# ZiyuanMa/MAPF_RL

Measured on NVIDIA B200. Metric: env_agent_steps_per_sec_step_observe, higher is better.
Workload: dtype u8

## Files before the change

mapf_rl_b200/csrc/mapf_bfs_device.cuh:

```cuda
#pragma once
#include <type_traits>

#include "mapf_common.cuh"

namespace {

#ifdef MAPF_ENABLE_DIAG
__device__ unsigned long long g_bfs_cycles[8];
#endif

template <int RW, int RPL>
struct BfsState {
    uint32_t unv[RPL][RW];
    uint32_t fro[RPL][RW];
    uint32_t m1[RPL][RW];
    uint32_t m2[RPL][RW];
};

__device__ __forceinline__ uint32_t bfs_column_mask(int L, int w)
{
    const int lo = max(4 - 32 * w, 0), hi = min(L + 4 - 32 * w, 32);
    if (hi <= lo) return 0u;
    return (hi - lo == 32) ? 0xffffffffu : (((1u << (hi - lo)) - 1u) << lo);
}

template <int RW, int RPL>
struct BfsFree {
    uint32_t v[RPL][RW];
};

template <int RW, int RPL, int APW>
__device__ __forceinline__ void bfs_load_free(const EnvDims &d, const uint32_t *ob, BfsFree<RW, RPL> &F)
{
    constexpr int LW = 32 / APW;
    const int lane = (threadIdx.x & 31) % LW;
#pragma unroll
    for (int q = 0; q < RPL; ++q) {
        const int row = lane * RPL + q;
#pragma unroll
        for (int w = 0; w < RW; ++w)
            F.v[q][w] = (row < d.L) ? (~__ldcg(ob + (row + 4) * d.RWS + w) & bfs_column_mask(d.L, w)) : 0u;
    }
}

template <int RW, int RPL, int APW>
__device__ __forceinline__ void bfs_init(const EnvDims &d, const BfsFree<RW, RPL> &F, const int gx, const int gy, const bool alive,
                                         BfsState<RW, RPL> &S)
{
    constexpr int LW = 32 / APW;
    const int lane = (threadIdx.x & 31) % LW;
#pragma unroll
    for (int q = 0; q < RPL; ++q) {
        const int row = lane * RPL + q;
#pragma unroll
        for (int w = 0; w < RW; ++w) {
            const uint32_t fre = alive ? F.v[q][w] : 0u;
            const int p = gy + 4;
            S.fro[q][w] = (row == gx && (p >> 5) == w) ? ((1u << (p & 31)) & fre) : 0u;
            S.unv[q][w] = fre & ~S.fro[q][w];
            S.m1[q][w] = S.m2[q][w] = 0;
        }
    }
}

template <int RW, int RPL, int APW, bool WRAP>
__device__ __forceinline__ uint32_t bfs_wave(const BfsState<RW, RPL> &S, uint32_t (&nw)[RPL][RW])
{
    constexpr int LW = 32 / APW;
    const int lane = (threadIdx.x & 31) % LW;
    uint32_t any = 0;
#pragma unroll
    for (int w = 0; w < RW; ++w) {
        uint32_t above, below;
        if constexpr (WRAP) {
            above = __shfl_sync(MAPF_FULL_MASK, S.fro[RPL - 1][w], (lane + LW - 1) & (LW - 1), LW);
            below = __shfl_sync(MAPF_FULL_MASK, S.fro[0][w], (lane + 1) & (LW - 1), LW);
        } else {
            above = __shfl_up_sync(MAPF_FULL_MASK, S.fro[RPL - 1][w], 1, LW);
            below = __shfl_down_sync(MAPF_FULL_MASK, S.fro[0][w], 1, LW);
            if (lane == 0) above = 0;
            if (lane == LW - 1) below = 0;
        }
#pragma unroll
        for (int q = 0; q < RPL; ++q) {
            const uint32_t f = S.fro[q][w];
            const uint32_t fl = w > 0 ? __funnelshift_l(S.fro[q][w > 0 ? w - 1 : 0], f, 1) : f << 1;
            const uint32_t fr = w < RW - 1 ? __funnelshift_r(f, S.fro[q][w < RW - 1 ? w + 1 : w], 1) : f >> 1;
            const uint32_t up = q > 0 ? S.fro[q > 0 ? q - 1 : 0][w] : above;
            const uint32_t dn = q < RPL - 1 ? S.fro[q < RPL - 1 ? q + 1 : q][w] : below;
            const uint32_t x = (fl | fr | up | dn) & S.unv[q][w];
            nw[q][w] = x;
            any |= x;
        }
    }
    return any;
}

template <int RW, int RPL, int SEL>
__device__ __forceinline__ void bfs_apply(BfsState<RW, RPL> &S, const uint32_t (&nw)[RPL][RW])
{
#pragma unroll
    for (int q = 0; q < RPL; ++q)
#pragma unroll
        for (int w = 0; w < RW; ++w) {
            S.unv[q][w] -= nw[q][w];
            S.fro[q][w] = nw[q][w];
            if constexpr (SEL == 1) S.m1[q][w] += nw[q][w];
            if constexpr (SEL == 2) S.m2[q][w] += nw[q][w];
        }
}

template <int RW, int RPL, int APW, bool KEEP>
__device__ __forceinline__ void bfs_emit(const EnvDims &d, const uint32_t *ob, const BfsFree<RW, RPL> &F, const int e, const int a,
                                         const bool alive, const BfsState<RW, RPL> &S, uint32_t *__restrict__ navi)
{
    constexpr int LW = 32 / APW;
    const int lane = (threadIdx.x & 31) % LW;
    uint32_t pl[4][RPL][RW];
    uint32_t z[RPL][RW];
#pragma unroll
    for (int q = 0; q < RPL; ++q) {
        const int row = alive ? lane * RPL + q : d.L;
#pragma unroll
        for (int w = 0; w < RW; ++w) {
            uint32_t fre;
            if constexpr (KEEP) fre = alive ? F.v[q][w] : 0u;
            else fre = (row < d.L) ? (~__ldcg(ob + (row + 4) * d.RWS + w) & bfs_column_mask(d.L, w)) : 0u;
            z[q][w] = fre & ~S.unv[q][w] & ~S.m1[q][w] & ~S.m2[q][w];
        }
    }
    auto closer = [](uint32_t c1, uint32_t c2, uint32_t cz, uint32_t n1, uint32_t n2, uint32_t nz) -> uint32_t {
        return (c1 & nz) | (c2 & n1) | (cz & n2);
    };
#pragma unroll
    for (int w = 0; w < RW; ++w) {
        uint32_t a1 = __shfl_up_sync(MAPF_FULL_MASK, S.m1[RPL - 1][w], 1, LW), b1 = __shfl_down_sync(MAPF_FULL_MASK, S.m1[0][w], 1, LW);
        uint32_t a2 = __shfl_up_sync(MAPF_FULL_MASK, S.m2[RPL - 1][w], 1, LW), b2 = __shfl_down_sync(MAPF_FULL_MASK, S.m2[0][w], 1, LW);
        uint32_t az = __shfl_up_sync(MAPF_FULL_MASK, z[RPL - 1][w], 1, LW), bz = __shfl_down_sync(MAPF_FULL_MASK, z[0][w], 1, LW);
        if (lane == 0) a1 = a2 = az = 0;
        if (lane == LW - 1) b1 = b2 = bz = 0;
#pragma unroll
        for (int q = 0; q < RPL; ++q) {
            auto left = [&](const uint32_t(&m)[RPL][RW]) {
                return w > 0 ? __funnelshift_l(m[q][w > 0 ? w - 1 : 0], m[q][w], 1) : m[q][w] << 1;
            };
            auto right = [&](const uint32_t(&m)[RPL][RW]) {
                return w < RW - 1 ? __funnelshift_r(m[q][w], m[q][w < RW - 1 ? w + 1 : w], 1) : m[q][w] >> 1;
            };
            const uint32_t c1 = S.m1[q][w], c2 = S.m2[q][w], cz = z[q][w];
            const uint32_t u1 = q > 0 ? S.m1[q > 0 ? q - 1 : 0][w] : a1, u2 = q > 0 ? S.m2[q > 0 ? q - 1 : 0][w] : a2,
                           uz = q > 0 ? z[q > 0 ? q - 1 : 0][w] : az;
            const uint32_t d1 = q < RPL - 1 ? S.m1[q < RPL - 1 ? q + 1 : q][w] : b1, d2 = q < RPL - 1 ? S.m2[q < RPL - 1 ? q + 1 : q][w] : b2,
                           dz = q < RPL - 1 ? z[q < RPL - 1 ? q + 1 : q][w] : bz;
            pl[0][q][w] = closer(c1, c2, cz, u1, u2, uz);
            pl[1][q][w] = closer(c1, c2, cz, d1, d2, dz);
            pl[2][q][w] = closer(c1, c2, cz, left(S.m1), left(S.m2), left(z));
            pl[3][q][w] = closer(c1, c2, cz, right(S.m1), right(S.m2), right(z));
        }
    }
    uint2 *nv = reinterpret_cast<uint2 *>(navi + ((size_t)e * d.N + a) * d.navi_agent_stride);
#pragma unroll
    for (int q = 0; q < RPL; ++q) {
        const int row = lane * RPL + q;
        if (row >= d.L || !alive) continue;
        const int pr = row + 4, bx1 = pr >> 3, r1 = pr & 7;
#pragma unroll
        for (int by = 0; by < 4 * RW; ++by) {
            if (by >= d.NB) continue;
            constexpr int kLast = RW - 1;
            const int w = by >> 2;
            const int s = (by & 3) * 8;
            uint32_t f[4];
#pragma unroll
            for (int k = 0; k < 4; ++k)
                f[k] = __funnelshift_r(pl[k][q][w], w < kLast ? pl[k][q][w < kLast ? w + 1 : kLast] : 0u, s) & 0xffffu;
            const uint2 v = make_uint2(f[0] | (f[1] << 16), f[2] | (f[3] << 16));
            if (bx1 < d.NB) nv[((size_t)(bx1 * d.NB + by) << 4) + r1] = v;
            if (bx1 > 0) nv[((size_t)((bx1 - 1) * d.NB + by) << 4) + r1 + 8] = v;
        }
    }
}

template <int RW, int RPL, int APW, bool WRAP, bool DIST, bool KEEP>
__device__ __forceinline__ void bfs_navi_search(const EnvDims &d, const int e, const int a, const int i, const bool alive,
                                                const uint32_t *__restrict__ ob, const BfsFree<RW, RPL> &F, const int gx, const int gy,
                                                uint32_t *__restrict__ navi, int32_t *__restrict__ dist_out)
{
    constexpr int LW = 32 / APW;
    const int lane = (threadIdx.x & 31) % LW;
#ifdef MAPF_ENABLE_DIAG
    const long long tb0 = clock64();
    long long triples = 0;
#endif
    BfsState<RW, RPL> S;
    bfs_init<RW, RPL, APW>(d, F, gx, gy, alive, S);
#ifdef MAPF_ENABLE_DIAG
    const long long tb1 = clock64();
#endif

    int32_t *dist = nullptr;
    if constexpr (DIST) {
        dist = alive ? dist_out + ((size_t)i * d.N + a) * d.L * d.L : nullptr;
        for (int q = 0; q < RPL; ++q) {
            const int row = lane * RPL + q;
            if (dist && row < d.L)
                for (int y = 0; y < d.L; ++y) dist[row * d.L + y] = MAPF_DIST_UNREACHABLE;
        }
        __syncwarp();
#pragma unroll
        for (int q = 0; q < RPL; ++q)
#pragma unroll
            for (int w = 0; w < RW; ++w)
                if (dist && S.fro[q][w]) dist[gx * d.L + gy] = 0;
    }

    auto wave = [&](auto selc, const int t) -> uint32_t {
        constexpr int sel = decltype(selc)::value;
        uint32_t nw[RPL][RW];
        const uint32_t any = bfs_wave<RW, RPL, APW, WRAP>(S, nw);
        bfs_apply<RW, RPL, sel>(S, nw);
        if constexpr (DIST) {
#pragma unroll
            for (int q = 0; q < RPL; ++q)
#pragma unroll
                for (int w = 0; w < RW; ++w) {
                    uint32_t x = dist ? nw[q][w] : 0u;
                    while (x) {
                        int b = __ffs(x) - 1;
                        x &= x - 1;
                        dist[(lane * RPL + q) * d.L + (32 * w + b - 4)] = t;
                    }
                }
        }
        return any;
    };
    for (int t = 1;; t += 3) {
        wave(std::integral_constant<int, 1>{}, t);
        wave(std::integral_constant<int, 2>{}, t + 1);
        const uint32_t any = wave(std::integral_constant<int, 0>{}, t + 2);
#ifdef MAPF_ENABLE_DIAG
        ++triples;
#endif
        if (!__any_sync(MAPF_FULL_MASK, any != 0)) break;
    }
#ifdef MAPF_ENABLE_DIAG
    const long long tb2 = clock64();
#endif
    bfs_emit<RW, RPL, APW, KEEP>(d, ob, F, e, a, alive, S, navi);
#ifdef MAPF_ENABLE_DIAG
    if (e == 0 && (threadIdx.x & 31) == 0) {
        const long long tb3 = clock64();
        atomicAdd(&g_bfs_cycles[0], (unsigned long long)(tb1 - tb0));
        atomicAdd(&g_bfs_cycles[1], (unsigned long long)(tb2 - tb1));
        atomicAdd(&g_bfs_cycles[2], (unsigned long long)(tb3 - tb2));
        atomicAdd(&g_bfs_cycles[3], 1ull);
        atomicAdd(&g_bfs_cycles[4], (unsigned long long)triples);
    }
#endif
}

template <int RW, int RPL, int APW>
__device__ __forceinline__ void bfs_navi_warp(const EnvDims &d, const int e, const int a, const int i, const bool alive,
                                              const uint32_t *__restrict__ obst, const uint8_t *__restrict__ goal,
                                              uint32_t *__restrict__ navi, int32_t *__restrict__ dist_out)
{
    constexpr int LW = 32 / APW;
    const uint32_t *ob = obst + (size_t)e * d.obst_stride;
    const uchar2 gg = __ldcg(reinterpret_cast<const uchar2 *>(goal) + (size_t)e * d.N + a);
    BfsFree<RW, RPL> F;
    bfs_load_free<RW, RPL, APW>(d, ob, F);
    if (dist_out) bfs_navi_search<RW, RPL, APW, false, true, false>(d, e, a, i, alive, ob, F, gg.x, gg.y, navi, dist_out);
    else if (d.L < LW * RPL) bfs_navi_search<RW, RPL, APW, true, false, false>(d, e, a, i, alive, ob, F, gg.x, gg.y, navi, nullptr);
    else bfs_navi_search<RW, RPL, APW, false, false, false>(d, e, a, i, alive, ob, F, gg.x, gg.y, navi, nullptr);
}

template <int RW, int RPL, int APW>
__device__ __forceinline__ void bfs_navi_warp_pre(const EnvDims &d, const int e, const int a, const bool alive, const uint32_t *__restrict__ ob,
                                                  const BfsFree<RW, RPL> &F, const int gx, const int gy, uint32_t *__restrict__ navi)
{
    constexpr int LW = 32 / APW;
    if (d.L < LW * RPL) bfs_navi_search<RW, RPL, APW, true, false, true>(d, e, a, 0, alive, ob, F, gx, gy, navi, nullptr);
    else bfs_navi_search<RW, RPL, APW, false, false, true>(d, e, a, 0, alive, ob, F, gx, gy, navi, nullptr);
}

}
```

mapf_rl_b200/csrc/mapf_reset_device.cuh:

```cuda
#pragma once
#include "mapf_common.cuh"

namespace {


__device__ __forceinline__ uint4 philox4x32_10(uint4 c, uint2 k)
{
#pragma unroll
    for (int r = 0; r < 10; ++r) {
        const uint32_t hi0 = __umulhi(0xD2511F53u, c.x), lo0 = 0xD2511F53u * c.x;
        const uint32_t hi1 = __umulhi(0xCD9E8D57u, c.z), lo1 = 0xCD9E8D57u * c.z;
        c = make_uint4(hi1 ^ c.y ^ k.x, lo1, hi0 ^ c.w ^ k.y, lo0);
        k.x += 0x9E3779B9u;
        k.y += 0xBB67AE85u;
    }
    return c;
}

enum : uint32_t { PURPOSE_DENSITY = 0, PURPOSE_MAP = 1, PURPOSE_AGENT = 2 };

#ifdef MAPF_ENABLE_DIAG
__device__ unsigned long long g_reset_cycles[8];
#define MAPF_RESET_TICK(slot)                 \
    do {                                      \
        const long long _now = clock64();     \
        _acc[slot] += _now - _t0;             \
        _t0 = _now;                           \
    } while (0)
#else
#define MAPF_RESET_TICK(slot) do {} while (0)
#endif

template <int RW, int RPL>
struct Bits {
    uint32_t v[RPL][RW];
};

template <int RW, int RPL>
__device__ __forceinline__ void dilate(const Bits<RW, RPL> &f, Bits<RW, RPL> &out, int lane)
{
#pragma unroll
    for (int q = 0; q < RPL; ++q)
#pragma unroll
        for (int w = 0; w < RW; ++w) {
            const uint32_t x = f.v[q][w];
            uint32_t fl = x << 1, fr = x >> 1;
            if (w > 0) fl |= f.v[q][w > 0 ? w - 1 : 0] >> 31;
            if (w < RW - 1) fr |= f.v[q][w < RW - 1 ? w + 1 : w] << 31;
            uint32_t up = __shfl_up_sync(MAPF_FULL_MASK, x, 1);
            uint32_t dn = __shfl_down_sync(MAPF_FULL_MASK, x, 1);
            uint32_t wrap_up = 0, wrap_dn = 0;
            if (q > 0) wrap_up = __shfl_sync(MAPF_FULL_MASK, f.v[q > 0 ? q - 1 : 0][w], 31);
            if (q < RPL - 1) wrap_dn = __shfl_sync(MAPF_FULL_MASK, f.v[q < RPL - 1 ? q + 1 : q][w], 0);
            if (lane == 0) up = wrap_up;
            if (lane == 31) dn = wrap_dn;
            out.v[q][w] = fl | fr | up | dn;
        }
}

template <int RW, int RPL>
__device__ __forceinline__ int count_bits(const Bits<RW, RPL> &m)
{
    int c = 0;
#pragma unroll
    for (int q = 0; q < RPL; ++q)
#pragma unroll
        for (int w = 0; w < RW; ++w) c += __popc(m.v[q][w]);
    return c;
}

__device__ __forceinline__ int nth_set_bit(uint32_t m, int n)
{
    int pos = 0;
#pragma unroll
    for (int half = 16; half >= 1; half >>= 1) {
        const int c = __popc(m & ((1u << half) - 1u));
        if (n >= c) {
            n -= c;
            pos += half;
            m >>= half;
        }
    }
    return pos;
}

template <int RW, int RPL>
__device__ __forceinline__ int pick_bit(const Bits<RW, RPL> &m, uint32_t rnd, int lane, int &total_out)
{
    constexpr int kMax = 32 * RW * RPL;
    constexpr int kBits = kMax >= 512 ? 10 : (kMax >= 256 ? 9 : (kMax >= 128 ? 8 : (kMax >= 64 ? 7 : 6)));
    const int c = count_bits(m);
    const uint32_t lt = (1u << lane) - 1u;
    int excl = 0, total = 0;
#pragma unroll
    for (int k = 0; k < kBits; ++k) {
        const uint32_t b = __ballot_sync(MAPF_FULL_MASK, (c >> k) & 1);
        excl += __popc(b & lt) << k;
        total += __popc(b) << k;
    }
    total_out = total;
    if (total == 0) return -1;
    const int r = (int)__umulhi(rnd, (uint32_t)total);
    int local = r - excl;
    uint32_t code = 0;
    if (local >= 0 && local < c) {
        bool found = false;
#pragma unroll
        for (int q = 0; q < RPL; ++q)
#pragma unroll
            for (int w = 0; w < RW; ++w) {
                const int pc = __popc(m.v[q][w]);
                if (!found && local < pc) {
                    code = (uint32_t)((((lane + 32 * q) << 8) | (32 * w + nth_set_bit(m.v[q][w], local))) + 1);
                    found = true;
                }
                if (!found) local -= pc;
            }
    }
    return (int)__reduce_or_sync(MAPF_FULL_MASK, code) - 1;
}

template <int RW, int RPL>
__device__ __forceinline__ void clear_cell(Bits<RW, RPL> &m, int code, int lane)
{
    const int row = code >> 8, col = code & 0xff;
#pragma unroll
    for (int q = 0; q < RPL; ++q)
#pragma unroll
        for (int w = 0; w < RW; ++w)
            if (lane + 32 * q == row && (col >> 5) == w) m.v[q][w] &= ~(1u << (col & 31));
}

template <int RW, int RPL>
__device__ __forceinline__ bool test_cell(const Bits<RW, RPL> &m, int code, int lane)
{
    const int row = code >> 8, col = code & 0xff;
    bool hit = false;
#pragma unroll
    for (int q = 0; q < RPL; ++q)
#pragma unroll
        for (int w = 0; w < RW; ++w)
            if (lane + 32 * q == row && (col >> 5) == w) hit = (m.v[q][w] >> (col & 31)) & 1u;
    return __any_sync(MAPF_FULL_MASK, hit);
}

template <int RW, int RPL>
__device__ __forceinline__ void reset_env_warp(const EnvDims &d, const int e, const uint64_t seed, const uint64_t g,
                                               const float density, uint32_t *__restrict__ obst, uint8_t *__restrict__ pos,
                                               uint8_t *__restrict__ goal, int32_t *__restrict__ steps, int32_t *__restrict__ err)
{
    const int lane = threadIdx.x & 31;
    const int L = d.L, N = d.N;
    const uint2 key = make_uint2((uint32_t)seed, (uint32_t)(seed >> 32));
    const uint32_t g_lo = (uint32_t)g, g_hi = (uint32_t)(g >> 32);

    float dens = density;
    if (density < 0.f) {
        const uint4 r = philox4x32_10(make_uint4(g_lo, g_hi, PURPOSE_DENSITY, 0u), key);
        const float u = (float)(r.x >> 8) * (1.0f / 16777216.0f);
        dens = u < 0.66f ? sqrtf(u * 0.5f * 0.33f) : 0.5f - sqrtf((1.0f - u) * 0.5f * 0.17f);
    }
    const uint32_t thresh = dens <= 0.f ? 0u : (dens >= 1.f ? 0xffffffffu : (uint32_t)((double)dens * 4294967296.0));

    Bits<RW, RPL> fre, elig, comp, big;
    int big_n = 0;
#ifdef MAPF_ENABLE_DIAG
    long long _t0 = clock64();
    long long _acc[8] = {0, 0, 0, 0, 0, 0, 0, 0};
#endif
    for (uint32_t attempt = 0;; ++attempt) {
        if (attempt >= 256) {
            if (lane == 0) atomicOr(err, MAPF_ERRBIT_RESET);
            break;
        }
#pragma unroll
        for (int q = 0; q < RPL; ++q) {
            const int row = lane + 32 * q;
#pragma unroll
            for (int w = 0; w < RW; ++w) fre.v[q][w] = 0;
            if (row < L) {
                for (int y4 = 0; y4 < L; y4 += 4) {
                    const uint4 r = philox4x32_10(make_uint4(g_lo, g_hi, PURPOSE_MAP | (attempt << 8), (uint32_t)(row * 64 + (y4 >> 2))), key);
                    uint32_t nib = (r.x >= thresh ? 1u : 0u) | (r.y >= thresh ? 2u : 0u) | (r.z >= thresh ? 4u : 0u) | (r.w >= thresh ? 8u : 0u);
                    if (y4 + 4 > L) nib &= (1u << (L - y4)) - 1u;
                    const int p = y4 + 4;
#pragma unroll
                    for (int w = 0; w < RW; ++w)
                        if ((p >> 5) == w) fre.v[q][w] |= nib << (p & 31);
                }
            }
        }
        MAPF_RESET_TICK(0);
        dilate(fre, elig, lane);
#pragma unroll
        for (int q = 0; q < RPL; ++q)
#pragma unroll
            for (int w = 0; w < RW; ++w) {
                elig.v[q][w] &= fre.v[q][w];
                comp.v[q][w] = 0;
                big.v[q][w] = 0;
            }
        big_n = 0;
        bool ok = true;
        MAPF_RESET_TICK(1);
        uint32_t draw_x[MAPF_MAX_AGENTS / 32], draw_y[MAPF_MAX_AGENTS / 32];
#pragma unroll
        for (int k = 0; k < MAPF_MAX_AGENTS / 32; ++k) {
            draw_x[k] = draw_y[k] = 0;
            if (k * 32 < N) {
                const uint4 r = philox4x32_10(make_uint4(g_lo, g_hi, PURPOSE_AGENT | (attempt << 8), (uint32_t)(k * 32 + lane)), key);
                draw_x[k] = r.x, draw_y[k] = r.y;
            }
        }
        for (int i = 0; i < N; ++i) {
            uint2 r = make_uint2(0u, 0u);
#pragma unroll
            for (int k = 0; k < MAPF_MAX_AGENTS / 32; ++k)
                if ((i >> 5) == k) r = make_uint2(__shfl_sync(MAPF_FULL_MASK, draw_x[k], i & 31), __shfl_sync(MAPF_FULL_MASK, draw_y[k], i & 31));
            MAPF_RESET_TICK(2);
            int total;
            const int s = pick_bit(elig, r.x, lane, total);
            MAPF_RESET_TICK(3);
            if (s < 0) {
                ok = false;
                break;
            }
            if (!test_cell(comp, s, lane) && big_n > 0 && test_cell(big, s, lane)) {
#pragma unroll
                for (int q = 0; q < RPL; ++q)
#pragma unroll
                    for (int w = 0; w < RW; ++w) comp.v[q][w] = big.v[q][w];
            } else if (!test_cell(comp, s, lane)) {
#pragma unroll
                for (int q = 0; q < RPL; ++q)
#pragma unroll
                    for (int w = 0; w < RW; ++w) comp.v[q][w] = 0;
                {
                    const int row = s >> 8, col = s & 0xff;
#pragma unroll
                    for (int q = 0; q < RPL; ++q)
#pragma unroll
                        for (int w = 0; w < RW; ++w)
                            if (lane + 32 * q == row && (col >> 5) == w) comp.v[q][w] = 1u << (col & 31);
                }
                for (;;) {
                    uint32_t grew = 0;
#pragma unroll
                    for (int rep = 0; rep < 4; ++rep) {
                        Bits<RW, RPL> nb;
                        dilate(comp, nb, lane);
                        grew = 0;
#pragma unroll
                        for (int q = 0; q < RPL; ++q)
#pragma unroll
                            for (int w = 0; w < RW; ++w) {
                                const uint32_t add = nb.v[q][w] & fre.v[q][w] & ~comp.v[q][w];
                                comp.v[q][w] |= add;
                                grew |= add;
                            }
                    }
                    if (!__any_sync(MAPF_FULL_MASK, grew != 0)) break;
                }
                const int n = __reduce_add_sync(MAPF_FULL_MASK, count_bits(comp));
                if (n > big_n) {
                    big_n = n;
#pragma unroll
                    for (int q = 0; q < RPL; ++q)
#pragma unroll
                        for (int w = 0; w < RW; ++w) big.v[q][w] = comp.v[q][w];
                }
            }
            MAPF_RESET_TICK(4);
            clear_cell(elig, s, lane);
            Bits<RW, RPL> cand;
#pragma unroll
            for (int q = 0; q < RPL; ++q)
#pragma unroll
                for (int w = 0; w < RW; ++w) cand.v[q][w] = elig.v[q][w] & comp.v[q][w];
            int cnt;
            const int t = pick_bit(cand, r.y, lane, cnt);
            clear_cell(elig, t, lane);
            if (cnt - 1 < 2) {
#pragma unroll
                for (int q = 0; q < RPL; ++q)
#pragma unroll
                    for (int w = 0; w < RW; ++w) elig.v[q][w] &= ~comp.v[q][w];
            }
            MAPF_RESET_TICK(5);
            if (lane == 0) {
                const size_t o = ((size_t)e * N + i) * 2;
                pos[o] = (uint8_t)(s >> 8);
                pos[o + 1] = (uint8_t)((s & 0xff) - 4);
                goal[o] = (uint8_t)(t >> 8);
                goal[o + 1] = (uint8_t)((t & 0xff) - 4);
            }
            MAPF_RESET_TICK(6);
        }
        if (ok) break;
    }

    uint32_t *ob = obst + (size_t)e * d.obst_stride;
    for (int w = lane; w < d.obst_stride; w += 32) {
        const int prow = w / d.RWS;
        if (prow < 4 || prow >= L + 4 || w - prow * d.RWS >= RW) ob[w] = 0;
    }
#pragma unroll
    for (int q = 0; q < RPL; ++q) {
        const int row = lane + 32 * q;
        if (row < L) {
#pragma unroll
            for (int w = 0; w < RW; ++w) {
                const int lo = max(4 - 32 * w, 0), hi = min(L + 4 - 32 * w, 32);
                uint32_t cm = 0;
                if (hi > lo) cm = (hi - lo == 32) ? 0xffffffffu : (((1u << (hi - lo)) - 1u) << lo);
                ob[(row + 4) * d.RWS + w] = ~fre.v[q][w] & cm;
            }
        }
    }
    if (lane == 0) steps[e] = 0;
#ifdef MAPF_ENABLE_DIAG
    MAPF_RESET_TICK(7);
    if (e == 0 && lane == 0)
        for (int i = 0; i < 8; ++i) g_reset_cycles[i] = (unsigned long long)_acc[i];
#endif
}

}
```

Baseline: 10.12 billion.

## Track eligible-cell counts incrementally in reset and use byte_perm for navi packing

Reset agent placement now keeps per-lane and warp-total counts of eligible and candidate cells and updates them as cells are cleared, instead of re-running the ballot-based popcount prefix on every pick. Component and biggest-component membership bits are returned with the picked cell, which removes the separate test_cell warp votes. The BFS navi output packing uses __byte_perm instead of funnel shifts and masks for byte-aligned offsets on larger grid configurations. The incremental bookkeeping is more intricate: lane ownership is decoded from the row with `& 31`, and counts must be invalidated exactly when the component changes.

```diff
diff --git a/mapf_rl_b200/csrc/mapf_bfs_device.cuh b/mapf_rl_b200/csrc/mapf_bfs_device.cuh
--- a/mapf_rl_b200/csrc/mapf_bfs_device.cuh
+++ b/mapf_rl_b200/csrc/mapf_bfs_device.cuh
@@ -169,12 +169,25 @@
             if (by >= d.NB) continue;
             constexpr int kLast = RW - 1;
             const int w = by >> 2;
-            const int s = (by & 3) * 8;
-            uint32_t f[4];
-#pragma unroll
-            for (int k = 0; k < 4; ++k)
-                f[k] = __funnelshift_r(pl[k][q][w], w < kLast ? pl[k][q][w < kLast ? w + 1 : kLast] : 0u, s) & 0xffffu;
-            const uint2 v = make_uint2(f[0] | (f[1] << 16), f[2] | (f[3] << 16));
+            constexpr bool kPermute = KEEP || RW * RPL > 9;
+            auto two = [&](const int k0, const int k1) -> uint32_t {
+                if constexpr (!kPermute) {
+                    const uint32_t f0 = __funnelshift_r(pl[k0][q][w], w < kLast ? pl[k0][q][w < kLast ? w + 1 : kLast] : 0u, (by & 3) * 8);
+                    const uint32_t f1 = __funnelshift_r(pl[k1][q][w], w < kLast ? pl[k1][q][w < kLast ? w + 1 : kLast] : 0u, (by & 3) * 8);
+                    return (f0 & 0xffffu) | (f1 << 16);
+                }
+                switch (by & 3) {
+                    case 0: return __byte_perm(pl[k0][q][w], pl[k1][q][w], 0x5410);
+                    case 1: return __byte_perm(pl[k0][q][w], pl[k1][q][w], 0x6521);
+                    case 2: return __byte_perm(pl[k0][q][w], pl[k1][q][w], 0x7632);
+                    default: {
+                        const uint32_t n0 = w < kLast ? pl[k0][q][w < kLast ? w + 1 : kLast] : 0u;
+                        const uint32_t n1 = w < kLast ? pl[k1][q][w < kLast ? w + 1 : kLast] : 0u;
+                        return __byte_perm(__funnelshift_r(pl[k0][q][w], n0, 24), __funnelshift_r(pl[k1][q][w], n1, 24), 0x5410);
+                    }
+                }
+            };
+            const uint2 v = make_uint2(two(0, 1), two(2, 3));
             if (bx1 < d.NB) nv[((size_t)(bx1 * d.NB + by) << 4) + r1] = v;
             if (bx1 > 0) nv[((size_t)((bx1 - 1) * d.NB + by) << 4) + r1 + 8] = v;
         }
diff --git a/mapf_rl_b200/csrc/mapf_reset_device.cuh b/mapf_rl_b200/csrc/mapf_reset_device.cuh
--- a/mapf_rl_b200/csrc/mapf_reset_device.cuh
+++ b/mapf_rl_b200/csrc/mapf_reset_device.cuh
@@ -84,8 +84,13 @@
     return pos;
 }
 
-template <int RW, int RPL>
-__device__ __forceinline__ int pick_bit(const Bits<RW, RPL> &m, uint32_t rnd, int lane, int &total_out)
+struct BitCount {
+    uint32_t ce;
+    int total;
+};
+
+template <int RW, int RPL>
+__device__ __forceinline__ BitCount count_set_bits(const Bits<RW, RPL> &m, int lane)
 {
     constexpr int kMax = 32 * RW * RPL;
     constexpr int kBits = kMax >= 512 ? 10 : (kMax >= 256 ? 9 : (kMax >= 128 ? 8 : (kMax >= 64 ? 7 : 6)));
@@ -98,26 +103,46 @@
         excl += __popc(b & lt) << k;
         total += __popc(b) << k;
     }
-    total_out = total;
-    if (total == 0) return -1;
-    const int r = (int)__umulhi(rnd, (uint32_t)total);
-    int local = r - excl;
-    uint32_t code = 0;
-    if (local >= 0 && local < c) {
-        bool found = false;
-#pragma unroll
-        for (int q = 0; q < RPL; ++q)
-#pragma unroll
-            for (int w = 0; w < RW; ++w) {
-                const int pc = __popc(m.v[q][w]);
-                if (!found && local < pc) {
-                    code = (uint32_t)((((lane + 32 * q) << 8) | (32 * w + nth_set_bit(m.v[q][w], local))) + 1);
-                    found = true;
-                }
-                if (!found) local -= pc;
-            }
-    }
-    return (int)__reduce_or_sync(MAPF_FULL_MASK, code) - 1;
+    return {(uint32_t)c | ((uint32_t)excl << 16), total};
+}
+
+__device__ __forceinline__ void count_cleared(BitCount &n, int code, int lane)
+{
+    const int owner = (code >> 8) & 31;
+    n.ce -= (uint32_t)(lane == owner) | ((uint32_t)(owner < lane) << 16);
+    n.total -= 1;
+}
+
+template <bool TAGS, int RW, int RPL>
+__device__ __forceinline__ int pick_bit(const Bits<RW, RPL> &m, const BitCount &n, uint32_t rnd, int lane, const Bits<RW, RPL> &t0,
+                                        const Bits<RW, RPL> &t1)
+{
+    const int r = (int)__umulhi(rnd, (uint32_t)n.total);
+    int local = r - (int)(n.ce >> 16);
+    const bool owner = local >= 0 && local < (int)(n.ce & 0xffffu);
+    bool found = false;
+    uint32_t sel = 0, s0 = 0, s1 = 0;
+    int at = 0;
+#pragma unroll
+    for (int q = 0; q < RPL; ++q)
+#pragma unroll
+        for (int w = 0; w < RW; ++w) {
+            const int pc = __popc(m.v[q][w]);
+            const bool take = !found && local < pc;
+            sel = take ? m.v[q][w] : sel;
+            if constexpr (TAGS) {
+                s0 = take ? t0.v[q][w] : s0;
+                s1 = take ? t1.v[q][w] : s1;
+            }
+            at = take ? (((lane + 32 * q) << 8) | (32 * w)) : at;
+            local -= (found || take) ? 0 : pc;
+            found |= take;
+        }
+    const int b = nth_set_bit(sel, local);
+    uint32_t code = owner ? (uint32_t)((at | b) + 1) : 0u;
+    if constexpr (TAGS) code |= owner ? ((((s0 >> b) & 1u) << 16) | (((s1 >> b) & 1u) << 17)) : 0u;
+    const uint32_t all = __reduce_or_sync(MAPF_FULL_MASK, code);
+    return (int)((all & 0xffffu) - 1u) | (int)(all & 0x30000u);
 }
 
 template <int RW, int RPL>
@@ -129,19 +154,6 @@
 #pragma unroll
         for (int w = 0; w < RW; ++w)
             if (lane + 32 * q == row && (col >> 5) == w) m.v[q][w] &= ~(1u << (col & 31));
-}
-
-template <int RW, int RPL>
-__device__ __forceinline__ bool test_cell(const Bits<RW, RPL> &m, int code, int lane)
-{
-    const int row = code >> 8, col = code & 0xff;
-    bool hit = false;
-#pragma unroll
-    for (int q = 0; q < RPL; ++q)
-#pragma unroll
-        for (int w = 0; w < RW; ++w)
-            if (lane + 32 * q == row && (col >> 5) == w) hit = (m.v[q][w] >> (col & 31)) & 1u;
-    return __any_sync(MAPF_FULL_MASK, hit);
 }
 
 template <int RW, int RPL>
@@ -212,25 +224,30 @@
                 draw_x[k] = r.x, draw_y[k] = r.y;
             }
         }
+        BitCount ne = count_set_bits(elig, lane), nc = {0u, 0};
+        bool nc_ok = false;
         for (int i = 0; i < N; ++i) {
             uint2 r = make_uint2(0u, 0u);
 #pragma unroll
             for (int k = 0; k < MAPF_MAX_AGENTS / 32; ++k)
                 if ((i >> 5) == k) r = make_uint2(__shfl_sync(MAPF_FULL_MASK, draw_x[k], i & 31), __shfl_sync(MAPF_FULL_MASK, draw_y[k], i & 31));
             MAPF_RESET_TICK(2);
-            int total;
-            const int s = pick_bit(elig, r.x, lane, total);
-            MAPF_RESET_TICK(3);
-            if (s < 0) {
+            if (ne.total == 0) {
                 ok = false;
                 break;
             }
-            if (!test_cell(comp, s, lane) && big_n > 0 && test_cell(big, s, lane)) {
+            const int sc = pick_bit<true>(elig, ne, r.x, lane, comp, big);
+            const int s = sc & 0xffff;
+            const bool in_comp = (sc >> 16) & 1, in_big = (sc >> 17) & 1;
+            MAPF_RESET_TICK(3);
+            if (!in_comp && in_big) {
 #pragma unroll
                 for (int q = 0; q < RPL; ++q)
 #pragma unroll
                     for (int w = 0; w < RW; ++w) comp.v[q][w] = big.v[q][w];
-            } else if (!test_cell(comp, s, lane)) {
+                nc_ok = false;
+            } else if (!in_comp) {
+                nc_ok = false;
 #pragma unroll
                 for (int q = 0; q < RPL; ++q)
 #pragma unroll
@@ -272,19 +289,30 @@
             }
             MAPF_RESET_TICK(4);
             clear_cell(elig, s, lane);
+            count_cleared(ne, s, lane);
             Bits<RW, RPL> cand;
 #pragma unroll
             for (int q = 0; q < RPL; ++q)
 #pragma unroll
                 for (int w = 0; w < RW; ++w) cand.v[q][w] = elig.v[q][w] & comp.v[q][w];
-            int cnt;
-            const int t = pick_bit(cand, r.y, lane, cnt);
+            if (nc_ok) {
+                count_cleared(nc, s, lane);
+            } else {
+                nc = count_set_bits(cand, lane);
+                nc_ok = true;
+            }
+            const int cnt = nc.total;
+            const int t = pick_bit<false>(cand, nc, r.y, lane, cand, cand);
             clear_cell(elig, t, lane);
+            count_cleared(ne, t, lane);
+            count_cleared(nc, t, lane);
             if (cnt - 1 < 2) {
 #pragma unroll
                 for (int q = 0; q < RPL; ++q)
 #pragma unroll
                     for (int w = 0; w < RW; ++w) elig.v[q][w] &= ~comp.v[q][w];
+                ne = count_set_bits(elig, lane);
+                nc_ok = false;
             }
             MAPF_RESET_TICK(5);
             if (lane == 0) {
```

Result: faster. 10.49 billion, median of 6 (+3.7%).
